# fxxJuses/MICFormer

Measured on AMD Instinct MI355X. Metric: train volumes/sec (128^3 CT+MRI pair), higher is better.
Workload: dtype bf16; 1 GPU; MicFormer base Head(embed_dim=48, depths 2-2-6-2, heads 3-6-12-24, window 2^3, 8 classes) full train step (fwd + MDiceLoss + bwd + Adam/cosine) on 128^3 CT+MR pairs, DropPath on; local_batch=2, global_batch=2, parallelism=dp1, launch=hipGraph replay (one graph)

## Files before the change

### micformer_amd/csrc/common.h

```cpp
#pragma once
#include <hip/hip_runtime.h>
#include <stdint.h>

#include "../../include/micformer_hip.h"
#include "gemm_core.h"

#define MICF_RETURN_LAUNCH()                          \
  do {                                                \
    return hipGetLastError() == hipSuccess ? MICF_OK : MICF_ELAUNCH; \
  } while (0)

namespace micf {

struct Options {
  int block_wave = 1;
  int block_recompute_h = 0;
  int block_debug = 0;
  int sample_tile = 1;
  int sample_e = -1;
  int cell_cap = -1;
  int tile_cap_hits = -1, tile_cap_cell = -1, tile_cap_voxel = -1;
};
Options& options();

struct Geo {
  int B, D, H, W;
  FastDiv fW, fH, fD;
  Geo() {}
  Geo(int B_, int D_, int H_, int W_) : B(B_), D(D_), H(H_), W(W_), fW((uint32_t)W_), fH((uint32_t)H_), fD((uint32_t)D_) {}
  __host__ __device__ int64_t tokens() const { return (int64_t)B * D * H * W; }
  __device__ __forceinline__ void decode(int t, int& b, int& d, int& h, int& w) const {
    uint32_t q, r;
    fW.divmod((uint32_t)t, q, r); w = (int)r;
    fH.divmod(q, q, r); h = (int)r;
    fD.divmod(q, q, r); d = (int)r; b = (int)q;
  }
  __device__ __forceinline__ int token(int b, int d, int h, int w) const { return ((b * D + d) * H + h) * W + w; }
};

__device__ __forceinline__ float wave_sum(float v) {
#pragma unroll
  for (int o = 32; o > 0; o >>= 1) v += __shfl_xor(v, o, 64);
  return v;
}

int colsum_atomic(const float* dy, const float* scale, int64_t rps, float* out, int64_t M, int N, hipStream_t s);

constexpr int kOffsetHidden = 16;
struct CellLists {
  int* count;
  int* ovf_count;
  int* list;
  int* ovf;
  int cap;
  float* w8;
};
struct SampleFwdSet { const float *h, *ln_g, *ln_b, *w1, *xa; float *flow, *xs; };
struct SampleBwdSet {
  const float *dxs, *h, *ln_g, *ln_b, *w1, *xa, *flow;
  float *dxa, *dh, *dln_g, *dln_b, *dw1;
  CellLists cl;
  float* partials;
};
int offset_sample_fwd_groups(const SampleFwdSet* sets, int n, int B, int D, int H, int W, int C, float eps, hipStream_t stream);
int offset_sample_bwd_groups(SampleBwdSet* sets, int n, int B, int D, int H, int W, int C, float eps, float* workspace,
                             int64_t workspace_floats, hipStream_t s, int phase = 0);
struct SampleFinishCall { const SampleBwdSet* sets; int n, B, D, H, W, C; float* workspace; int64_t workspace_floats; };
int offset_sample_finish_many(const SampleFinishCall* calls, int ncalls, hipStream_t s);

struct Conv3FwdSet { const float* x1; const float* x2; const float* w; const float* bias; float* y; float* wt; };
struct Conv3BwdSet { const float* dy; const float* w; float* wt; float* dx1; float* dx2; };
int conv3_fwd_x_groups(const Conv3FwdSet* sets, int n, int c1, int c2, int B, int D, int H, int W, int N, hipStream_t stream, int dtype,
                       int prepared, int y_zeroed);
bool conv3_fwd_x_splits(int B, int D, int H, int W, int c1, int c2);
int conv3_bwd_data_x_groups(const Conv3BwdSet* sets, int ng, int c1, int acc1, int c2, int acc2, int B, int D, int H, int W, int N,
                            hipStream_t stream, int dtype, int prepared);

int conv3_bwd_data_x(const float* dy, const float* w, float* wt, float* dx1, int c1, int acc1, float* dx2, int c2, int acc2, int B,
                     int D, int H, int W, int N, hipStream_t stream, int dtype = 0, int prepared = 0);

int64_t conv3_fwdx_workspace(int N, int c1, int c2);
int conv3_fwd_x(const float* x1, int c1, const float* x2, int c2, const float* w, const float* bias, float* y, float* wt, int B, int D,
                int H, int W, int N, hipStream_t stream, int dtype = 0, int prepared = 0);
int64_t conv3_wgradx_workspace(int B, int D, int H, int W, int N, int c1, int c2, int items = 1);
int conv3_wgradx_items(const float* const* dy, const float* const* x1, const float* const* x2, float* const* dw, float* const* dbias,
                       int n, int c1, int c2, int B, int D, int H, int W, int N, float* ws, int64_t ws_floats, hipStream_t stream,
                       int dtype);
int conv3_wgradx(const float* dy, const float* x1, int c1, const float* x2, int c2, float* dw, float* dbias, int B, int D, int H,
                 int W, int N, float* ws, int64_t ws_floats, hipStream_t stream, int dtype = 0);

}
```

### micformer_amd/csrc/conv3_bwdx.hip

```cpp
#include <cstdlib>
#include "common.h"
#include "conv3_layout.h"
#include "gemm_dma.h"

namespace micf {

constexpr int xKS = 20;

struct BwdxArgs {
  const float* dy; int N;
  const float* wt;
  float* d1; float* d2; int oc1, oc2, acc1, acc2;
  int O;
  int B, D, H, W, tiles_d, tiles_h, tiles_w, ngroups;
  const float* dyb; const float* wtb; float* d1b; float* d2b;
};

__global__ void __launch_bounds__(256) conv3_wt_kernel(const float* __restrict__ w, float* __restrict__ wt, int N, int Cin) {
  const int64_t id = (int64_t)blockIdx.x * 256 + threadIdx.x;
  if (id < conv3_bwd_layout_items(Cin)) conv3_bwd_layout_write(w, wt, N, Cin, id);
}

template <int TW, int NCT, bool BF16>
__global__ void __launch_bounds__(256) conv3_bwdx_kernel(BwdxArgs a) {
  constexpr int CH = 16 / TW, TH = 4 * CH, TD = 2;
  constexpr int HD = TD + 2, HH = TH + 2, HW = TW + 2, HALO = HD * HH * HW;
  __shared__ __attribute__((aligned(16))) float Xs[HALO * xKS];
  if (blockIdx.z) { a.dy = a.dyb; a.wt = a.wtb; a.d1 = a.d1b; a.d2 = a.d2b; }
  const int tid = threadIdx.x, lane = tid & 63, wave = __builtin_amdgcn_readfirstlane(tid >> 6), li = lane & 15, lr = lane >> 4;
  int q = blockIdx.x;
  if (gridDim.x >= 64 && (gridDim.x & 7) == 0) q = (q & 7) * (gridDim.x >> 3) + (q >> 3);
  const int tw = q % a.tiles_w; q /= a.tiles_w;
  const int th = q % a.tiles_h; q /= a.tiles_h;
  const int td = q % a.tiles_d; const int b = q / a.tiles_d;
  const int d0 = td * TD, h0 = th * TH, w0 = tw * TW;
  const int64_t DHW = (int64_t)a.D * a.H * a.W;
  const int ct0 = blockIdx.y * NCT;
  const int nct = min(NCT, a.O / 16 - ct0);

  {
    constexpr int NH = (HALO * 4 + 255) / 256;
    float4 hv4[NH];
#pragma unroll
    for (int it = 0; it < NH; ++it) {
      const int idx = tid + it * 256;
      hv4[it] = make_float4(0.f, 0.f, 0.f, 0.f);
      if (idx < HALO * 4) {
        const int hv = idx >> 2, g = idx & 3;
        const int hw = hv % HW, hh = (hv / HW) % HH, hd = hv / (HW * HH);
        const int dd = d0 + hd - 1, yy = h0 + hh - 1, ww = w0 + hw - 1;
        if ((unsigned)dd < (unsigned)a.D && (unsigned)yy < (unsigned)a.H && (unsigned)ww < (unsigned)a.W && 4 * g < a.N)
          hv4[it] = *reinterpret_cast<const float4*>(a.dy + ((int64_t)b * DHW + ((int64_t)dd * a.H + yy) * a.W + ww) * a.N + 4 * g);
      }
    }
#pragma unroll
    for (int it = 0; it < NH; ++it) {
      const int idx = tid + it * 256;
      if (idx < HALO * 4) {
        if constexpr (BF16)
          *reinterpret_cast<uint2*>(&reinterpret_cast<uint16_t*>(Xs)[(idx >> 2) * xKS + 4 * (idx & 3)]) =
              make_uint2(pack_bf16(hv4[it].x, hv4[it].y), pack_bf16(hv4[it].z, hv4[it].w));
        else
          *reinterpret_cast<float4*>(&Xs[(idx >> 2) * xKS + 4 * (idx & 3)]) = hv4[it];
      }
    }
  }
  int ld[2], lh[2], lw[2];
#pragma unroll
  for (int tj = 0; tj < 2; ++tj) {
    const int ct = 2 * wave + tj;
    ld[tj] = ct / 4;
    lh[tj] = (ct % 4) * CH + li / TW;
    lw[tj] = li % TW;
  }
  f32x4 acc[NCT][2];
#pragma unroll
  for (int t = 0; t < NCT; ++t) { acc[t][0] = f32x4{0.f, 0.f, 0.f, 0.f}; acc[t][1] = f32x4{0.f, 0.f, 0.f, 0.f}; }
  const float* wp = a.wt + ((int64_t)(ct0 * 16 + li)) * 16 + 4 * lr;
  const int64_t tap_stride = (int64_t)a.O * 16;
  if constexpr (BF16) {
    typedef unsigned u32x4 __attribute__((ext_vector_type(4)));
    const uint16_t* Xh = reinterpret_cast<const uint16_t*>(Xs);
    const u32x4* wq = reinterpret_cast<const u32x4*>(reinterpret_cast<const uint16_t*>(a.wt + conv3_bwd_layout_f32(a.O)) +
                                                     (((int64_t)(ct0 * 16 + li)) * 4 + lr) * 8);
    const int64_t pair_stride = (int64_t)a.O * 4;
// ... 64 lines not shown
  for (int t = 0; t < NCT; ++t) av[t] = (t < nct && !BF16) ? *reinterpret_cast<const float4*>(wp + t * 256) : make_float4(0.f, 0.f, 0.f, 0.f);
  if constexpr (!BF16) __syncthreads();
#pragma unroll 1
  for (int tap = 0; tap < (BF16 ? 0 : 27); ++tap) {
    if (tap + 1 < 27) {
#pragma unroll
      for (int t = 0; t < NCT; ++t)
        an[t] = (t < nct) ? *reinterpret_cast<const float4*>(wp + (tap + 1) * tap_stride + t * 256) : make_float4(0.f, 0.f, 0.f, 0.f);
    }
    const int kd = tap / 9, kh = (tap / 3) % 3, kw = tap % 3;
    float4 bv[2];
#pragma unroll
    for (int tj = 0; tj < 2; ++tj) {
      const int zd = ld[tj] + 2 - kd, zh = lh[tj] + 2 - kh, zw = lw[tj] + 2 - kw;
      bv[tj] = *reinterpret_cast<const float4*>(&Xs[((zd * HH + zh) * HW + zw) * xKS + 4 * lr]);
    }
    if constexpr (!BF16) {
#pragma unroll
      for (int s = 0; s < 4; ++s) {
        const float b0 = s == 0 ? bv[0].x : (s == 1 ? bv[0].y : (s == 2 ? bv[0].z : bv[0].w));
        const float b1 = s == 0 ? bv[1].x : (s == 1 ? bv[1].y : (s == 2 ? bv[1].z : bv[1].w));
#pragma unroll
        for (int t = 0; t < NCT; ++t) {
          const float av_s = s == 0 ? av[t].x : (s == 1 ? av[t].y : (s == 2 ? av[t].z : av[t].w));
          acc[t][0] = __builtin_amdgcn_mfma_f32_16x16x4f32(av_s, b0, acc[t][0], 0, 0, 0);
          acc[t][1] = __builtin_amdgcn_mfma_f32_16x16x4f32(av_s, b1, acc[t][1], 0, 0, 0);
        }
      }
    } else {
      if ((tap & 1) || tap == 26) {
        const float4 z = make_float4(0.f, 0.f, 0.f, 0.f);
        const bool pair = tap & 1;
        const bf16x8 bb0 = pair ? to_bf16x8(bprev[0], bv[0]) : to_bf16x8(bv[0], z);
        const bf16x8 bb1 = pair ? to_bf16x8(bprev[1], bv[1]) : to_bf16x8(bv[1], z);
#pragma unroll
        for (int t = 0; t < NCT; ++t) {
          const bf16x8 ba = pair ? to_bf16x8(aprev[t], av[t]) : to_bf16x8(av[t], z);
          acc[t][0] = __builtin_amdgcn_mfma_f32_16x16x32_bf16(ba, bb0, acc[t][0], 0, 0, 0);
          acc[t][1] = __builtin_amdgcn_mfma_f32_16x16x32_bf16(ba, bb1, acc[t][1], 0, 0, 0);
        }
      } else {
        bprev[0] = bv[0]; bprev[1] = bv[1];
#pragma unroll
        for (int t = 0; t < NCT; ++t) aprev[t] = av[t];
      }
    }
#pragma unroll
    for (int t = 0; t < NCT; ++t) av[t] = an[t];
  }
#pragma unroll
  for (int tj = 0; tj < 2; ++tj) {
    const int dd = d0 + ld[tj], yy = h0 + lh[tj], ww = w0 + lw[tj];
    if (dd >= a.D || yy >= a.H || ww >= a.W) continue;
    const int64_t tok = (int64_t)b * DHW + ((int64_t)dd * a.H + yy) * a.W + ww;
    auto where = [&](int t, int& accf) -> float* {
      const int c = (ct0 + t) * 16 + 4 * lr;
      if (t >= nct) return nullptr;
      if (c < a.oc1) { accf = a.acc1; return a.d1 ? a.d1 + tok * a.oc1 + c : nullptr; }
      accf = a.acc2;
      return a.d2 ? a.d2 + tok * a.oc2 + (c - a.oc1) : nullptr;
    };
    constexpr int EB = NCT >= 6 ? 2 : NCT;
#pragma unroll
    for (int t0 = 0; t0 < NCT; t0 += EB) {
      float4 old[EB];
#pragma unroll
      for (int u = 0; u < EB; ++u) {
        int accf = 0;
        const float* p = where(t0 + u, accf);
        old[u] = (p && accf) ? *reinterpret_cast<const float4*>(p) : make_float4(0.f, 0.f, 0.f, 0.f);
      }
#pragma unroll
      for (int u = 0; u < EB; ++u) {
        int accf = 0;
        float* p = where(t0 + u, accf);
        if (!p) continue;
        const f32x4 v = acc[t0 + u][tj];
        *reinterpret_cast<float4*>(p) = make_float4(v[0] + old[u].x, v[1] + old[u].y, v[2] + old[u].z, v[3] + old[u].w);
      }
    }
  }
}

template <int TW, bool BF16>
static hipError_t launch_bwdx(BwdxArgs& a, hipStream_t stream) {
  constexpr int CH = 16 / TW, TH = 4 * CH;
  a.tiles_d = (a.D + 1) / 2;
  a.tiles_h = (a.H + TH - 1) / TH;
  a.tiles_w = (a.W + TW - 1) / TW;
  const int64_t blocks = (int64_t)a.B * a.tiles_d * a.tiles_h * a.tiles_w;
  const int cts = a.O / 16;
  if (blocks * ((cts + 5) / 6) >= 128)
    hipLaunchKernelGGL((conv3_bwdx_kernel<TW, 6, BF16>), dim3((unsigned)blocks, (cts + 5) / 6, a.ngroups), dim3(256), 0, stream, a);
  else
    hipLaunchKernelGGL((conv3_bwdx_kernel<TW, 2, BF16>), dim3((unsigned)blocks, (cts + 1) / 2, a.ngroups), dim3(256), 0, stream, a);
  return hipGetLastError();
}

int conv3_bwd_data_x(const float* dy, const float* w, float* wt, float* dx1, int c1, int acc1, float* dx2, int c2, int acc2, int B,
                     int D, int H, int W, int N, hipStream_t stream, int dtype, int prepared) {
  const Conv3BwdSet one{dy, w, wt, dx1, dx2};
  return conv3_bwd_data_x_groups(&one, 1, c1, acc1, c2, acc2, B, D, H, W, N, stream, dtype, prepared);
}

int conv3_bwd_data_x_groups(const Conv3BwdSet* sets, int ng, int c1, int acc1, int c2, int acc2, int B, int D, int H, int W, int N,
                            hipStream_t stream, int dtype, int prepared) {
  if (!sets || ng < 1 || ng > 2) return MICF_EINVAL;
  const int O = c1 + c2;
  if (N > 16 || (N & 3) || (O & 15) || (c1 & 3) || (c2 & 3) || W < 4) return MICF_EUNSUPPORTED;
  for (int i = 0; i < ng; ++i)
    if (!aligned16(sets[i].dy) || !aligned16(sets[i].wt) || (sets[i].dx1 && !aligned16(sets[i].dx1)) || (sets[i].dx2 && !aligned16(sets[i].dx2)) ||
        (!sets[i].dx1) != (!sets[0].dx1) || (!sets[i].dx2) != (!sets[0].dx2))
      return MICF_EUNSUPPORTED;
  const float *dy = sets[0].dy;
  float *wt = sets[0].wt, *dx1 = sets[0].dx1, *dx2 = sets[0].dx2;
  const int64_t n = conv3_bwd_layout_items(O);
  if (!prepared) {
    for (int i = 0; i < ng; ++i) {
      hipLaunchKernelGGL(conv3_wt_kernel, dim3((unsigned)((n + 255) / 256)), dim3(256), 0, stream, sets[i].w, sets[i].wt, N, O);
      if (hipGetLastError() != hipSuccess) return MICF_ELAUNCH;
    }
  }
  BwdxArgs a{};
  a.dyb = sets[ng - 1].dy; a.wtb = sets[ng - 1].wt; a.d1b = sets[ng - 1].dx1; a.d2b = sets[ng - 1].dx2; a.ngroups = ng;
  a.dy = dy; a.N = N; a.wt = wt; a.d1 = dx1; a.d2 = dx2; a.oc1 = c1; a.oc2 = c2; a.acc1 = acc1; a.acc2 = acc2; a.O = O;
  a.B = B; a.D = D; a.H = H; a.W = W;
  const hipError_t e = dtype == MICF_DTYPE_BF16 ? ((W >= 12) ? launch_bwdx<16, true>(a, stream) : launch_bwdx<8, true>(a, stream))
                                                 : ((W >= 12) ? launch_bwdx<16, false>(a, stream) : launch_bwdx<8, false>(a, stream));
  return e == hipSuccess ? MICF_OK : MICF_ELAUNCH;
}

}
```

### micformer_amd/csrc/conv3_fwdx.hip

```cpp
#include <cstdlib>
#include "common.h"
#include "conv3_layout.h"
#include "gemm_dma.h"

namespace micf {

constexpr int fKS = 20;
constexpr int fAhead = 3;

struct FwdxArgs {
  const float* x1; const float* x2; int c1, c2;
  const float* wt;
  const float* bias; float* y; int N;
  const float* x1b; const float* x2b; const float* wtb; const float* biasb; float* yb;
  int B, D, H, W, tiles_d, tiles_h, tiles_w;
  int chunks, chunks_per_block;
};

__global__ void __launch_bounds__(256) conv3_wtf_kernel(const float* __restrict__ w, float* __restrict__ wt, int N, int Cin, int chunks) {
  const int64_t id = (int64_t)blockIdx.x * 256 + threadIdx.x;
  if (id < conv3_fwd_layout_items(Cin)) conv3_fwd_layout_write(w, wt, N, Cin, id);
}

template <int TW, bool BF16>
__global__ void __launch_bounds__(256) conv3_fwdx_kernel(FwdxArgs a) {
  constexpr int CH = 16 / TW, TH = 4 * CH, TD = 2;
  constexpr int HD = TD + 2, HH = TH + 2, HW = TW + 2, HALO = HD * HH * HW;
  constexpr int NH = (HALO * 4 + 255) / 256;
  __shared__ __attribute__((aligned(16))) float Xs[HALO * fKS];
  if (blockIdx.z) { a.x1 = a.x1b; a.x2 = a.x2b; a.wt = a.wtb; a.bias = a.biasb; a.y = a.yb; }
  const int tid = threadIdx.x, lane = tid & 63, wave = __builtin_amdgcn_readfirstlane(tid >> 6), li = lane & 15, lr = lane >> 4;
  int q = blockIdx.x;
  if (gridDim.x >= 64 && (gridDim.x & 7) == 0) q = (q & 7) * (gridDim.x >> 3) + (q >> 3);
  const int tw = q % a.tiles_w; q /= a.tiles_w;
  const int th = q % a.tiles_h; q /= a.tiles_h;
  const int td = q % a.tiles_d; const int b = q / a.tiles_d;
  const int d0 = td * TD, h0 = th * TH, w0 = tw * TW;
  const int64_t DHW = (int64_t)a.D * a.H * a.W;
  const int Cin = a.c1 + a.c2;
  const int kc_begin = blockIdx.y * a.chunks_per_block;
  const int kc_end = min(a.chunks, kc_begin + a.chunks_per_block);

  auto fetch = [&](int kc, float4 (&hv)[NH]) {
#pragma unroll
    for (int it = 0; it < NH; ++it) {
      const int idx = tid + it * 256;
      hv[it] = make_float4(0.f, 0.f, 0.f, 0.f);
      if (idx < HALO * 4) {
        const int v = idx >> 2, g = idx & 3;
        const int hw = v % HW, hh = (v / HW) % HH, hd = v / (HW * HH);
        const int dd = d0 + hd - 1, yy = h0 + hh - 1, ww = w0 + hw - 1;
        const int c = kc * 16 + 4 * g;
        if ((unsigned)dd < (unsigned)a.D && (unsigned)yy < (unsigned)a.H && (unsigned)ww < (unsigned)a.W && c < Cin) {
          const int64_t tok = (int64_t)b * DHW + ((int64_t)dd * a.H + yy) * a.W + ww;
          hv[it] = c < a.c1 ? *reinterpret_cast<const float4*>(a.x1 + tok * a.c1 + c)
                            : *reinterpret_cast<const float4*>(a.x2 + tok * a.c2 + (c - a.c1));
        }
      }
    }
  };
  uint16_t* Xh = reinterpret_cast<uint16_t*>(Xs);
  auto commit = [&](const float4 (&hv)[NH]) {
#pragma unroll
    for (int it = 0; it < NH; ++it) {
      const int idx = tid + it * 256;
      if (idx < HALO * 4) {
        if constexpr (BF16)
          *reinterpret_cast<uint2*>(&Xh[(idx >> 2) * fKS + 4 * (idx & 3)]) = make_uint2(pack_bf16(hv[it].x, hv[it].y), pack_bf16(hv[it].z, hv[it].w));
        else
          *reinterpret_cast<float4*>(&Xs[(idx >> 2) * fKS + 4 * (idx & 3)]) = hv[it];
      }
    }
  };

  int vbase[2];
#pragma unroll
  for (int tj = 0; tj < 2; ++tj) {
    const int ct = 2 * wave + tj;
    const int ld = ct / 4, lh = (ct % 4) * CH + li / TW, lw = li % TW;
    vbase[tj] = ((ld * HH + lh) * HW + lw) * fKS + 4 * lr;
  }
  f32x4 acc[2] = {f32x4{0.f, 0.f, 0.f, 0.f}, f32x4{0.f, 0.f, 0.f, 0.f}};
  float4 hv[NH];
  fetch(kc_begin, hv);
  for (int kc = kc_begin; kc < kc_end; ++kc) {
// ... 17 lines not shown
#pragma unroll
        for (int e = 0; e < 2; ++e) {
          const int tap = 2 * p + e;
          if (tap < 27) {
            const int kd = tap / 9, kh = (tap / 3) % 3, kw = tap % 3;
            const int off = ((kd * HH + kh) * HW + kw) * fKS;
            h[e][0] = *reinterpret_cast<const uint2*>(&Xh[vbase[0] + off]);
            h[e][1] = *reinterpret_cast<const uint2*>(&Xh[vbase[1] + off]);
          } else {
            h[e][0] = make_uint2(0u, 0u); h[e][1] = h[e][0];
          }
        }
        const u32x4 q0 = {h[0][0].x, h[0][0].y, h[1][0].x, h[1][0].y}, q1 = {h[0][1].x, h[0][1].y, h[1][1].x, h[1][1].y};
        acc[0] = __builtin_amdgcn_mfma_f32_16x16x32_bf16(__builtin_bit_cast(bf16x8, aq), __builtin_bit_cast(bf16x8, q0), acc[0], 0, 0, 0);
        acc[1] = __builtin_amdgcn_mfma_f32_16x16x32_bf16(__builtin_bit_cast(bf16x8, aq), __builtin_bit_cast(bf16x8, q1), acc[1], 0, 0, 0);
      }
      continue;
    }
    float4 ring[fAhead + 1];
    float4 aprev = make_float4(0.f, 0.f, 0.f, 0.f);
    uint2 hprev0 = make_uint2(0u, 0u), hprev1 = hprev0;
#pragma unroll
    for (int t = 0; t < fAhead; ++t) ring[t] = *reinterpret_cast<const float4*>(wp + t * 256);
#pragma unroll
    for (int tap = 0; tap < 27; ++tap) {
      if (tap + fAhead < 27) ring[(tap + fAhead) % (fAhead + 1)] = *reinterpret_cast<const float4*>(wp + (tap + fAhead) * 256);
      const float4 av = ring[tap % (fAhead + 1)];
      const int kd = tap / 9, kh = (tap / 3) % 3, kw = tap % 3;
      const int off = ((kd * HH + kh) * HW + kw) * fKS;
      if constexpr (!BF16) {
        const float4 b0 = *reinterpret_cast<const float4*>(&Xs[vbase[0] + off]);
        const float4 b1 = *reinterpret_cast<const float4*>(&Xs[vbase[1] + off]);
        acc[0] = __builtin_amdgcn_mfma_f32_16x16x4f32(av.x, b0.x, acc[0], 0, 0, 0);
        acc[1] = __builtin_amdgcn_mfma_f32_16x16x4f32(av.x, b1.x, acc[1], 0, 0, 0);
        acc[0] = __builtin_amdgcn_mfma_f32_16x16x4f32(av.y, b0.y, acc[0], 0, 0, 0);
        acc[1] = __builtin_amdgcn_mfma_f32_16x16x4f32(av.y, b1.y, acc[1], 0, 0, 0);
        acc[0] = __builtin_amdgcn_mfma_f32_16x16x4f32(av.z, b0.z, acc[0], 0, 0, 0);
        acc[1] = __builtin_amdgcn_mfma_f32_16x16x4f32(av.z, b1.z, acc[1], 0, 0, 0);
        acc[0] = __builtin_amdgcn_mfma_f32_16x16x4f32(av.w, b0.w, acc[0], 0, 0, 0);
        acc[1] = __builtin_amdgcn_mfma_f32_16x16x4f32(av.w, b1.w, acc[1], 0, 0, 0);
      } else {
        typedef unsigned u32x4 __attribute__((ext_vector_type(4)));
        const uint2 h0 = *reinterpret_cast<const uint2*>(&Xh[vbase[0] + off]);
        const uint2 h1 = *reinterpret_cast<const uint2*>(&Xh[vbase[1] + off]);
        if ((tap & 1) || tap == 26) {
          const float4 z = make_float4(0.f, 0.f, 0.f, 0.f);
          const bool pair = tap & 1;
          const bf16x8 ba = pair ? to_bf16x8(aprev, av) : to_bf16x8(av, z);
          const u32x4 q0 = pair ? u32x4{hprev0.x, hprev0.y, h0.x, h0.y} : u32x4{h0.x, h0.y, 0u, 0u};
          const u32x4 q1 = pair ? u32x4{hprev1.x, hprev1.y, h1.x, h1.y} : u32x4{h1.x, h1.y, 0u, 0u};
          acc[0] = __builtin_amdgcn_mfma_f32_16x16x32_bf16(ba, __builtin_bit_cast(bf16x8, q0), acc[0], 0, 0, 0);
          acc[1] = __builtin_amdgcn_mfma_f32_16x16x32_bf16(ba, __builtin_bit_cast(bf16x8, q1), acc[1], 0, 0, 0);
        } else {
          aprev = av; hprev0 = h0; hprev1 = h1;
        }
      }
    }
  }
  const bool atomic_out = gridDim.y > 1;
  const int n0 = 4 * lr;
#pragma unroll
  for (int tj = 0; tj < 2; ++tj) {
    const int ct = 2 * wave + tj;
    const int dd = d0 + ct / 4, yy = h0 + (ct % 4) * CH + li / TW, ww = w0 + li % TW;
    if (dd >= a.D || yy >= a.H || ww >= a.W || n0 >= a.N) continue;
    float* p = a.y + ((int64_t)b * DHW + ((int64_t)dd * a.H + yy) * a.W + ww) * a.N + n0;
    f32x4 v = acc[tj];
    if (a.bias && blockIdx.y == 0) {
#pragma unroll
      for (int e = 0; e < 4; ++e) if (n0 + e < a.N) v[e] += a.bias[n0 + e];
    }
    if (atomic_out) {
#pragma unroll
      for (int e = 0; e < 4; ++e) if (n0 + e < a.N) atomicAdd(p + e, v[e]);
    } else if (n0 + 3 < a.N && (a.N & 3) == 0) {
      *reinterpret_cast<float4*>(p) = make_float4(v[0], v[1], v[2], v[3]);
    } else {
#pragma unroll
      for (int e = 0; e < 4; ++e) if (n0 + e < a.N) p[e] = v[e];
    }
  }
}

int64_t conv3_fwdx_workspace(int N, int c1, int c2) {
  if (N <= 0 || N > 16 || c1 + c2 <= 0) return 0;
  return conv3_fwd_layout_floats(c1 + c2);
}

int conv3_fwd_x(const float* x1, int c1, const float* x2, int c2, const float* w, const float* bias, float* y, float* wt, int B, int D,
                int H, int W, int N, hipStream_t stream, int dtype, int prepared) {
  const Conv3FwdSet one{x1, x2, w, bias, y, wt};
  return conv3_fwd_x_groups(&one, 1, c1, c2, B, D, H, W, N, stream, dtype, prepared, 0);
}

bool conv3_fwd_x_splits(int B, int D, int H, int W, int c1, int c2) {
  const int chunks = (c1 + c2 + 15) / 16;
  const int tw_ = W >= 12 ? 16 : 8, th_ = 4 * (16 / tw_);
  const int64_t blocks = (int64_t)B * ((D + 1) / 2) * ((H + th_ - 1) / th_) * ((W + tw_ - 1) / tw_);
  return blocks < 256 && chunks > 1;
}

int conv3_fwd_x_groups(const Conv3FwdSet* sets, int n, int c1, int c2, int B, int D, int H, int W, int N, hipStream_t stream, int dtype,
                       int prepared, int y_zeroed) {
  if (!sets || n < 1 || n > 2) return MICF_EINVAL;
  if (N > 16 || (c1 & 3) || (c2 & 3) || W < 4) return MICF_EUNSUPPORTED;
  for (int i = 0; i < n; ++i)
    if (!aligned16(sets[i].x1) || (sets[i].x2 && !aligned16(sets[i].x2)) || !aligned16(sets[i].y) || !aligned16(sets[i].wt)) return MICF_EUNSUPPORTED;
  const float *x1 = sets[0].x1, *x2 = sets[0].x2, *w = sets[0].w, *bias = sets[0].bias;
  float *y = sets[0].y, *wt = sets[0].wt;
  const int Cin = c1 + c2, chunks = (Cin + 15) / 16;
  const int64_t nw = conv3_fwd_layout_items(Cin);
  if (!prepared) {
    for (int i = 0; i < n; ++i) {
      hipLaunchKernelGGL(conv3_wtf_kernel, dim3((unsigned)((nw + 255) / 256)), dim3(256), 0, stream, sets[i].w, sets[i].wt, N, Cin, chunks);
      if (hipGetLastError() != hipSuccess) return MICF_ELAUNCH;
    }
  }
  FwdxArgs a{};
  a.x1 = x1; a.x2 = x2 ? x2 : x1; a.c1 = c1; a.c2 = c2; a.wt = wt; a.bias = bias; a.y = y; a.N = N;
  a.B = B; a.D = D; a.H = H; a.W = W; a.chunks = chunks;
  const Conv3FwdSet& sb = sets[n - 1];
  a.x1b = sb.x1; a.x2b = sb.x2 ? sb.x2 : sb.x1; a.wtb = sb.wt; a.biasb = sb.bias; a.yb = sb.y;
  const int tw_ = W >= 12 ? 16 : 8, th_ = 4 * (16 / tw_);
  a.tiles_d = (D + 1) / 2; a.tiles_h = (H + th_ - 1) / th_; a.tiles_w = (W + tw_ - 1) / tw_;
  const int64_t blocks = (int64_t)B * a.tiles_d * a.tiles_h * a.tiles_w;
  int ysplit = 1;
  constexpr int split_target = 128;
  if (blocks < 256) { ysplit = (int)((split_target + blocks - 1) / blocks); if (ysplit > chunks) ysplit = chunks; if (ysplit < 1) ysplit = 1; }
  a.chunks_per_block = (chunks + ysplit - 1) / ysplit;
  ysplit = (chunks + a.chunks_per_block - 1) / a.chunks_per_block;
  if (ysplit > 1 && !y_zeroed)
    for (int i = 0; i < n; ++i)
      if (hipMemsetAsync(sets[i].y, 0, sizeof(float) * (size_t)B * D * H * W * N, stream) != hipSuccess) return MICF_ELAUNCH;
  const dim3 grid((unsigned)blocks, ysplit, n);
  if (dtype == MICF_DTYPE_BF16) {
    if (tw_ == 16) hipLaunchKernelGGL((conv3_fwdx_kernel<16, true>), grid, dim3(256), 0, stream, a);
    else hipLaunchKernelGGL((conv3_fwdx_kernel<8, true>), grid, dim3(256), 0, stream, a);
  } else {
    if (tw_ == 16) hipLaunchKernelGGL((conv3_fwdx_kernel<16, false>), grid, dim3(256), 0, stream, a);
    else hipLaunchKernelGGL((conv3_fwdx_kernel<8, false>), grid, dim3(256), 0, stream, a);
  }
  return hipGetLastError() == hipSuccess ? MICF_OK : MICF_ELAUNCH;
}

}
```

### micformer_amd/csrc/misc.hip

```cpp
#include <hip/hip_fp16.h>

#include "common.h"
#include <string.h>

namespace micf {

__global__ void __launch_bounds__(256) pad3d_kernel(const float* __restrict__ src, float* __restrict__ dst, int B, int D, int H,
                                                    int W, int Dp, int Hp, int Wp, int C, int64_t total) {
  for (int64_t i = (int64_t)blockIdx.x * 256 + threadIdx.x; i < total; i += (int64_t)gridDim.x * 256) {
    int64_t t = i / C; const int c = (int)(i - t * C);
    const int w = (int)(t % Wp); t /= Wp; const int h = (int)(t % Hp); t /= Hp; const int d = (int)(t % Dp); const int b = (int)(t / Dp);
    dst[i] = (d < D && h < H && w < W) ? src[((((int64_t)b * D + d) * H + h) * W + w) * C + c] : 0.f;
  }
}
__global__ void __launch_bounds__(256) crop3d_kernel(const float* __restrict__ src, float* __restrict__ dst, int B, int D, int H,
                                                     int W, int Dp, int Hp, int Wp, int C, int accumulate, int64_t total) {
  for (int64_t i = (int64_t)blockIdx.x * 256 + threadIdx.x; i < total; i += (int64_t)gridDim.x * 256) {
    int64_t t = i / C; const int c = (int)(i - t * C);
    const int w = (int)(t % W); t /= W; const int h = (int)(t % H); t /= H; const int d = (int)(t % D); const int b = (int)(t / D);
    const float v = src[((((int64_t)b * Dp + d) * Hp + h) * Wp + w) * C + c];
    dst[i] = accumulate ? dst[i] + v : v;
  }
}

__device__ __forceinline__ void ac_coord(int o, int Sin, int Sout, int& i0, int& i1, float& f) {
  const float scale = Sout > 1 ? (float)(Sin - 1) / (float)(Sout - 1) : 0.f;
  const float s = scale * (float)o;
  i0 = (int)s; if (i0 > Sin - 1) i0 = Sin - 1;
  i1 = i0 + (i0 < Sin - 1 ? 1 : 0);
  f = s - (float)i0;
}
template <bool BWD>
__global__ void __launch_bounds__(256) resize_kernel(const float* __restrict__ a, float* __restrict__ o, int B, int D, int H, int W,
                                                     int Do, int Ho, int Wo, int C, int64_t total) {
  for (int64_t i = (int64_t)blockIdx.x * 256 + threadIdx.x; i < total; i += (int64_t)gridDim.x * 256) {
    int64_t t = i / C; const int c = (int)(i - t * C);
    const int w = (int)(t % Wo); t /= Wo; const int h = (int)(t % Ho); t /= Ho; const int d = (int)(t % Do); const int b = (int)(t / Do);
    int d0, d1, h0, h1, w0, w1; float fd, fh, fw;
    ac_coord(d, D, Do, d0, d1, fd); ac_coord(h, H, Ho, h0, h1, fh); ac_coord(w, W, Wo, w0, w1, fw);
    float acc = 0.f;
    const float gv = BWD ? a[i] : 0.f;
#pragma unroll
    for (int q = 0; q < 8; ++q) {
      const int dd = (q & 4) ? d1 : d0, hh = (q & 2) ? h1 : h0, ww = (q & 1) ? w1 : w0;
      const float wt = ((q & 4) ? fd : 1.f - fd) * ((q & 2) ? fh : 1.f - fh) * ((q & 1) ? fw : 1.f - fw);
      const int64_t s = ((((int64_t)b * D + dd) * H + hh) * W + ww) * C + c;
      if (BWD) atomicAdd(o + s, wt * gv); else acc += wt * a[s];
    }
    if (!BWD) o[i] = acc;
  }
}

}
using namespace micf;

extern "C" int micf_abi_version(void) { return MICF_ABI_VERSION; }

micf::Options& micf::options() {
  static Options o;
  return o;
}

static int* option_slot(const char* name) {
  if (!name) return nullptr;
  Options& o = micf::options();
  const struct { const char* n; int* v; } table[] = {
      {"block_wave", &o.block_wave}, {"block_recompute_h", &o.block_recompute_h}, {"block_debug", &o.block_debug},
      {"sample_tile", &o.sample_tile}, {"sample_e", &o.sample_e}, {"cell_cap", &o.cell_cap},
      {"tile_cap_hits", &o.tile_cap_hits}, {"tile_cap_cell", &o.tile_cap_cell}, {"tile_cap_voxel", &o.tile_cap_voxel}};
  for (const auto& e : table)
    if (!strcmp(name, e.n)) return e.v;
  return nullptr;
}

extern "C" int micf_set_option(const char* name, int value) {
  int* slot = option_slot(name);
  if (!slot) return MICF_EINVAL;
  *slot = value;
  return MICF_OK;
}

extern "C" int micf_get_option(const char* name, int* value) {
  const int* slot = option_slot(name);
  if (!slot || !value) return MICF_EINVAL;
  *value = *slot;
  return MICF_OK;
}

extern "C" const char* micf_strerror(int code) {
  switch (code) {
    case MICF_OK: return "ok";
    case MICF_EINVAL: return "invalid argument (null pointer, bad size or misaligned buffer)";
    case MICF_EUNSUPPORTED: return "shape not supported by the HIP kernels";
    case MICF_ELAUNCH: return "HIP kernel launch failed";
    default: return "unknown micf error code";
  }
}

static int grid_for(int64_t total) { int64_t b = (total + 255) / 256; return (int)(b > 16384 ? 16384 : (b < 1 ? 1 : b)); }

extern "C" int micf_pad3d(const float* src, float* dst, int B, int D, int H, int W, int Dp, int Hp, int Wp, int C,
                          micf_stream_t stream) {
  if (!src || !dst || B <= 0 || D <= 0 || H <= 0 || W <= 0 || C <= 0 || Dp < D || Hp < H || Wp < W) return MICF_EINVAL;
  const int64_t total = (int64_t)B * Dp * Hp * Wp * C;
  hipLaunchKernelGGL(pad3d_kernel, dim3(grid_for(total)), dim3(256), 0, (hipStream_t)stream, src, dst, B, D, H, W, Dp, Hp, Wp, C, total);
  MICF_RETURN_LAUNCH();
}
extern "C" int micf_crop3d(const float* src, float* dst, int B, int D, int H, int W, int Dp, int Hp, int Wp, int C, int accumulate,
                           micf_stream_t stream) {
  if (!src || !dst || B <= 0 || D <= 0 || H <= 0 || W <= 0 || C <= 0 || Dp < D || Hp < H || Wp < W) return MICF_EINVAL;
  const int64_t total = (int64_t)B * D * H * W * C;
  hipLaunchKernelGGL(crop3d_kernel, dim3(grid_for(total)), dim3(256), 0, (hipStream_t)stream, src, dst, B, D, H, W, Dp, Hp, Wp, C,
                     accumulate, total);
  MICF_RETURN_LAUNCH();
}
extern "C" int micf_resize_trilinear_fwd(const float* src, float* dst, int B, int D, int H, int W, int Do, int Ho, int Wo, int C,
                                         micf_stream_t stream) {
  if (!src || !dst || B <= 0 || D <= 0 || H <= 0 || W <= 0 || Do <= 0 || Ho <= 0 || Wo <= 0 || C <= 0) return MICF_EINVAL;
  const int64_t total = (int64_t)B * Do * Ho * Wo * C;
  hipLaunchKernelGGL(resize_kernel<false>, dim3(grid_for(total)), dim3(256), 0, (hipStream_t)stream, src, dst, B, D, H, W, Do, Ho, Wo, C, total);
  MICF_RETURN_LAUNCH();
}
extern "C" int micf_resize_trilinear_bwd(const float* ddst, float* dsrc, int B, int D, int H, int W, int Do, int Ho, int Wo, int C,
                                         micf_stream_t stream) {
  if (!ddst || !dsrc || B <= 0 || D <= 0 || H <= 0 || W <= 0 || Do <= 0 || Ho <= 0 || Wo <= 0 || C <= 0) return MICF_EINVAL;
  hipStream_t s = (hipStream_t)stream;
  if (hipMemsetAsync(dsrc, 0, sizeof(float) * (size_t)B * D * H * W * C, s) != hipSuccess) return MICF_ELAUNCH;
  const int64_t total = (int64_t)B * Do * Ho * Wo * C;
  hipLaunchKernelGGL(resize_kernel<true>, dim3(grid_for(total)), dim3(256), 0, s, ddst, dsrc, B, D, H, W, Do, Ho, Wo, C, total);
  MICF_RETURN_LAUNCH();
}

extern "C" int micf_zero(void* p, int64_t bytes, micf_stream_t stream) {
  if (!p || bytes < 0) return MICF_EINVAL;
  if (bytes == 0) return MICF_OK;
  return hipMemsetAsync(p, 0, (size_t)bytes, (hipStream_t)stream) == hipSuccess ? MICF_OK : MICF_ELAUNCH;
}

namespace micf {
__device__ __forceinline__ uint64_t mix64(uint64_t z) {
  z += 0x9E3779B97F4A7C15ull;
  z = (z ^ (z >> 30)) * 0xBF58476D1CE4E5B9ull;
  z = (z ^ (z >> 27)) * 0x94D049BB133111EBull;
  return z ^ (z >> 31);
}
__global__ void __launch_bounds__(256) drop_path_draw_kernel(uint64_t* __restrict__ rng, const float* __restrict__ keep,
                                                             float* __restrict__ out, int n, int B) {
  const uint64_t seed = rng[0], ctr = rng[1];
  for (int e = threadIdx.x; e < n * B; e += 256) {
    const float k = keep[e / B];
    const uint64_t h = mix64(mix64(seed ^ mix64(ctr)) + (uint64_t)e);
    const float u = (float)(h >> 40) * (1.0f / 16777216.0f);
// ... 239 lines not shown
```

Before: 243.2 pairs/s.

## Add depth-marching 3x3x3 conv forward and backward-data kernels with LDS plane ring

Adds new conv3 forward and backward-data kernels. Each workgroup owns a 4x16 spatial footprint and marches along depth, keeping a three-plane bf16 halo ring in LDS, so each input plane is fetched once and reused across the three kd taps. Weights are held in registers for the whole march and the 27 taps are fed as MFMA 16x16x32 bf16 with double-buffered LDS reads. A plan header splits depth into ranges so the grid fills the chip and orders units for XCD locality. The new path is chosen automatically when bf16, N==16 and the grid is large enough, with a fallback to the old kernels and an option to disable it; the risks are lower occupancy from the larger LDS and extra synchronisation per depth step.

After: 243.5 pairs/s (median of 3 runs). No clear change (+0.1%).

```diff
diff --git a/micformer_amd/csrc/common.h b/micformer_amd/csrc/common.h
--- a/micformer_amd/csrc/common.h
+++ b/micformer_amd/csrc/common.h
@@ -20,6 +20,9 @@
   int sample_e = -1;
   int cell_cap = -1;
   int tile_cap_hits = -1, tile_cap_cell = -1, tile_cap_voxel = -1;
+  int conv3_march = -1;
+  int conv3_march_dcap = -1;
+  int conv3_march_last = 0;
 };
 Options& options();
 
diff --git a/micformer_amd/csrc/conv3_bwdx.hip b/micformer_amd/csrc/conv3_bwdx.hip
--- a/micformer_amd/csrc/conv3_bwdx.hip
+++ b/micformer_amd/csrc/conv3_bwdx.hip
@@ -1,6 +1,7 @@
 #include <cstdlib>
 #include "common.h"
 #include "conv3_layout.h"
+#include "conv3_march_plan.h"
 #include "gemm_dma.h"
 
 namespace micf {
@@ -231,6 +232,166 @@
   }
 }
 
+namespace mp = micf_march;
+constexpr int mDYB = 40;
+constexpr int mThreads = 64 * mp::kWaves;
+
+struct BwdMarchArgs {
+  const float* dy; const float* wt; float* d1; float* d2;
+  const float* dyb; const float* wtb; float* d1b; float* d2b;
+  int oc1, oc2, acc1, acc2, O;
+  mp::Plan plan;
+};
+
+__global__ void __launch_bounds__(mThreads, 3) conv3_bwdx_march_kernel(BwdMarchArgs a) {
+  typedef unsigned u32x4 __attribute__((ext_vector_type(4)));
+  constexpr int HW = mp::kHaloW, PL = mp::kPlaneRows, PLB = PL * mDYB;
+  constexpr int NQ = PL * 4;
+  constexpr int NB = (NQ + mThreads - 1) / mThreads;
+  __shared__ __attribute__((aligned(16))) char ring[3 * PLB];
+  if (blockIdx.z) { a.dy = a.dyb; a.wt = a.wtb; a.d1 = a.d1b; a.d2 = a.d2b; }
+  const int tid = threadIdx.x, lane = tid & 63, wave = __builtin_amdgcn_readfirstlane(tid >> 6), li = lane & 15, lr = lane >> 4;
+  const mp::Unit un = mp::decode(a.plan, blockIdx.x);
+  const int D = a.plan.D, H = a.plan.H, W = a.plan.W, h0 = un.h0, w0 = un.w0;
+  const int64_t tok0 = (int64_t)un.b * D * H * W;
+  const int tile = blockIdx.y * mp::kWaves + wave;
+  const bool active = tile * 16 < a.O;
+
+  const float* fsrc[NB];
+  unsigned fdst[NB];
+  unsigned fok = 0u;
+#pragma unroll
+  for (int u = 0; u < NB; ++u) {
+    const int idx = u * mThreads + tid, hv = idx >> 2, g = idx & 3;
+    const int yy = h0 + hv / HW - 1, ww = w0 + hv % HW - 1;
+    const bool ok = idx < NQ && (unsigned)yy < (unsigned)H && (unsigned)ww < (unsigned)W;
+    fsrc[u] = a.dy + (tok0 + (ok ? (int64_t)yy * W + ww : 0)) * 16 + 4 * g;
+    fdst[u] = (unsigned)(hv * mDYB + 8 * g);
+    fok |= ok ? 1u << u : 0u;
+  }
+  const int64_t fstride = (int64_t)H * W * 16;
+  auto fetch = [&](int dd, float4 (&v)[NB]) {
+    if ((unsigned)dd < (unsigned)D) {
+#pragma unroll
+      for (int u = 0; u < NB; ++u) v[u] = *reinterpret_cast<const float4*>(fsrc[u] + dd * fstride);
+    } else {
+#pragma unroll
+      for (int u = 0; u < NB; ++u) v[u] = make_float4(0.f, 0.f, 0.f, 0.f);
+    }
+  };
+  auto commit = [&](int slot, const float4 (&v)[NB]) {
+#pragma unroll
+    for (int u = 0; u < NB; ++u)
+      if (u * mThreads + tid < NQ) {
+        const bool ok = (fok >> u) & 1u;
+        *reinterpret_cast<uint2*>(ring + slot * PLB + fdst[u]) =
+            ok ? make_uint2(pack_bf16(v[u].x, v[u].y), pack_bf16(v[u].z, v[u].w)) : make_uint2(0u, 0u);
+      }
+  };
+
+  float4 va[NB], vb[NB];
+  int sc = un.d0 % 3;
+  {
+    float4 p0[NB], p1[NB];
+    fetch(un.d0 - 1, p0);
+    fetch(un.d0, p1);
+    fetch(un.d0 + 1, va);
+    if (un.d0 + 1 < un.d1) fetch(un.d0 + 2, vb);
+    commit(sc == 0 ? 2 : sc - 1, p0);
+    commit(sc, p1);
+  }
+  u32x4 aq[14];
+  {
+    const u32x4 zq = {0u, 0u, 0u, 0u};
+    const u32x4* wq = reinterpret_cast<const u32x4*>(reinterpret_cast<const uint16_t*>(a.wt + conv3_bwd_layout_f32(a.O))) +
+                      (((int64_t)(active ? tile : 0) * 16 + li) * 4 + lr);
+    const int64_t pair_stride = (int64_t)a.O * 4;
+#pragma unroll
+    for (int p = 0; p < 14; ++p) aq[p] = active ? wq[p * pair_stride] : zq;
+  }
+  float* outp = nullptr;
+  int ocw = 0, oacc = 0;
+  if (active && w0 + li < W) {
+    const int c = tile * 16 + 4 * lr;
+    const int64_t t = tok0 + (int64_t)h0 * W + w0 + li;
+    if (c < a.oc1) { ocw = a.oc1; oacc = a.acc1; outp = a.d1 ? a.d1 + t * a.oc1 + c : nullptr; }
+    else { ocw = a.oc2; oacc = a.acc2; outp = a.d2 ? a.d2 + t * a.oc2 + (c - a.oc1) : nullptr; }
+  }
+  const int64_t orow = (int64_t)W * ocw;
+  const unsigned lbase = (unsigned)(li * mDYB + 8 * lr);
+
+  auto step = [&](int d, float4 (&v)[NB]) {
+    const int sp = sc == 0 ? 2 : sc - 1, sn = sc == 2 ? 0 : sc + 1;
+    __syncthreads();
+    commit(sn, v);
+    __syncthreads();
+    if (d + 2 < un.d1) fetch(d + 3, v);
+    if (active) {
+      float* const op = outp ? outp + (int64_t)d * H * orow : nullptr;
+      float4 old[mp::kFootH];
+#pragma unroll
+      for (int j = 0; j < mp::kFootH; ++j) {
+        old[j] = make_float4(0.f, 0.f, 0.f, 0.f);
+        if (op && oacc && h0 + j < H) old[j] = *reinterpret_cast<const float4*>(op + j * orow);
+      }
+      const char* pk[3] = {ring + sn * PLB + lbase, ring + sc * PLB + lbase, ring + sp * PLB + lbase};
+      f32x4 acc[mp::kFootH];
+#pragma unroll
+      for (int j = 0; j < mp::kFootH; ++j) acc[j] = f32x4{0.f, 0.f, 0.f, 0.f};
+      auto read_stage = [&](int st, u32x4 (&bq)[2]) {
+        const int p = st >> 1;
+#pragma unroll
+        for (int jj = 0; jj < 2; ++jj) {
+          const int j = 2 * (st & 1) + jj;
+          uint2 h[2];
+#pragma unroll
+          for (int e = 0; e < 2; ++e) {
+            const int tap = 2 * p + e;
+            h[e] = make_uint2(0u, 0u);
+            if (tap < 27) {
+              const int kd = tap / 9, kh = (tap / 3) % 3, kw = tap % 3;
+              h[e] = *reinterpret_cast<const uint2*>(pk[kd] + ((j + 2 - kh) * HW + 2 - kw) * mDYB);
+            }
+          }
+          bq[jj] = u32x4{h[0].x, h[0].y, h[1].x, h[1].y};
+        }
+      };
+      u32x4 bq[2][2];
+      read_stage(0, bq[0]);
+#pragma unroll
+      for (int st = 0; st < 28; ++st) {
+        if (st + 1 < 28) read_stage(st + 1, bq[(st + 1) & 1]);
+#pragma unroll
+        for (int jj = 0; jj < 2; ++jj) {
+          const int j = 2 * (st & 1) + jj;
+          acc[j] = __builtin_amdgcn_mfma_f32_16x16x32_bf16(__builtin_bit_cast(bf16x8, aq[st >> 1]), __builtin_bit_cast(bf16x8, bq[st & 1][jj]), acc[j], 0, 0, 0);
+        }
+        __builtin_amdgcn_sched_barrier(0);
+      }
+      if (op) {
+#pragma unroll
+        for (int j = 0; j < mp::kFootH; ++j)
+          if (h0 + j < H)
+            *reinterpret_cast<float4*>(op + j * orow) =
+                make_float4(acc[j][0] + old[j].x, acc[j][1] + old[j].y, acc[j][2] + old[j].z, acc[j][3] + old[j].w);
+      }
+    }
+    sc = sn;
+  };
+  for (int d = un.d0; d < un.d1; d += 2) {
+    step(d, va);
+    if (d + 1 < un.d1) step(d + 1, vb);
+  }
+}
+
+static bool bwdx_marches(int ng, int O, int B, int D, int H, int W, int N, int dtype, mp::Plan& plan, int& ysplit) {
+  const Options& opt = options();
+  if (dtype != MICF_DTYPE_BF16 || opt.conv3_march == 0 || N != 16 || (int64_t)H * W * O > 0x7fffffffll) return false;
+  ysplit = (O / 16 + mp::kWaves - 1) / mp::kWaves;
+  plan = mp::make_plan(B, D, H, W, ng * ysplit, opt.conv3_march_dcap);
+  return opt.conv3_march == 1 || (W >= 12 && mp::fills_chip(plan, ng * ysplit));
+}
+
 template <int TW, bool BF16>
 static hipError_t launch_bwdx(BwdxArgs& a, hipStream_t stream) {
   constexpr int CH = 16 / TW, TH = 4 * CH;
@@ -270,6 +431,20 @@
       if (hipGetLastError() != hipSuccess) return MICF_ELAUNCH;
     }
   }
+  options().conv3_march_last = 0;
+  {
+    BwdMarchArgs m{};
+    int ysplit = 1;
+    if (bwdx_marches(ng, O, B, D, H, W, N, dtype, m.plan, ysplit)) {
+      m.dy = dy; m.wt = wt; m.d1 = dx1; m.d2 = dx2;
+      m.dyb = sets[ng - 1].dy; m.wtb = sets[ng - 1].wt; m.d1b = sets[ng - 1].dx1; m.d2b = sets[ng - 1].dx2;
+      m.oc1 = c1; m.oc2 = c2; m.acc1 = acc1; m.acc2 = acc2; m.O = O;
+      hipLaunchKernelGGL(conv3_bwdx_march_kernel, dim3((unsigned)m.plan.units, ysplit, ng), dim3(mThreads), 0, stream, m);
+      if (hipGetLastError() != hipSuccess) return MICF_ELAUNCH;
+      options().conv3_march_last = 1;
+      return MICF_OK;
+    }
+  }
   BwdxArgs a{};
   a.dyb = sets[ng - 1].dy; a.wtb = sets[ng - 1].wt; a.d1b = sets[ng - 1].dx1; a.d2b = sets[ng - 1].dx2; a.ngroups = ng;
   a.dy = dy; a.N = N; a.wt = wt; a.d1 = dx1; a.d2 = dx2; a.oc1 = c1; a.oc2 = c2; a.acc1 = acc1; a.acc2 = acc2; a.O = O;
diff --git a/micformer_amd/csrc/conv3_fwdx.hip b/micformer_amd/csrc/conv3_fwdx.hip
--- a/micformer_amd/csrc/conv3_fwdx.hip
+++ b/micformer_amd/csrc/conv3_fwdx.hip
@@ -1,6 +1,8 @@
 #include <cstdlib>
+#include <mutex>
 #include "common.h"
 #include "conv3_layout.h"
+#include "conv3_march_plan.h"
 #include "gemm_dma.h"
 
 namespace micf {
@@ -184,6 +186,180 @@
   }
 }
 
+namespace mp = micf_march;
+template <int NW> constexpr int mf_red_bytes() { return (NW / 2) * mp::kFootH * 64 * 16; }
+template <int NW> constexpr int mf_row_bytes() { return 2 * 16 * NW + 16; }
+template <int NW> constexpr int mf_lds_bytes() { return 3 * mp::kPlaneRows * mf_row_bytes<NW>() + mf_red_bytes<NW>(); }
+
+struct FwdMarchArgs {
+  const float* x1; const float* x2; const float* wt; const float* bias; float* y;
+  const float* x1b; const float* x2b; const float* wtb; const float* biasb; float* yb;
+  int c1, c2;
+  mp::Plan plan;
+};
+
+template <int NW>
+__global__ void __launch_bounds__(64 * NW, 3) conv3_fwdx_march_kernel(FwdMarchArgs a) {
+  typedef unsigned u32x4 __attribute__((ext_vector_type(4)));
+  constexpr int HW = mp::kHaloW, PL = mp::kPlaneRows, RS = mf_row_bytes<NW>(), PLB = PL * RS, mfThreads = 64 * NW;
+  constexpr int NB = (PL * 4 * NW + mfThreads - 1) / mfThreads;
+  extern __shared__ __attribute__((aligned(16))) char mf_smem[];
+  char* const ring = mf_smem;
+  float4* const red = reinterpret_cast<float4*>(mf_smem + 3 * PLB);
+  if (blockIdx.z) { a.x1 = a.x1b; a.x2 = a.x2b; a.wt = a.wtb; a.bias = a.biasb; a.y = a.yb; }
+  const int tid = threadIdx.x, lane = tid & 63, wave = __builtin_amdgcn_readfirstlane(tid >> 6), li = lane & 15, lr = lane >> 4;
+  const mp::Unit un = mp::decode(a.plan, blockIdx.x);
+  const int D = a.plan.D, H = a.plan.H, W = a.plan.W, h0 = un.h0, w0 = un.w0;
+  const int64_t tok0 = (int64_t)un.b * D * H * W;
+  const int Cin = a.c1 + a.c2, chunks = Cin >> 4;
+
+  const int G = Cin >> 2, RP = mfThreads / G, g = tid % G, r0 = tid / G;
+  const bool first = 4 * g < a.c1;
+  const int cw = first ? a.c1 : a.c2;
+  const float* const fbase = (first ? a.x1 + 4 * g : a.x2 + (4 * g - a.c1)) + tok0 * cw;
+  const int64_t fstride = (int64_t)H * W * cw;
+  const unsigned fdst = (unsigned)(r0 * RS + 8 * g);
+  unsigned foff[NB];
+  unsigned fok = 0u;
+#pragma unroll
+  for (int u = 0; u < NB; ++u) {
+    const int hv = u * RP + r0;
+    const int yy = h0 + hv / HW - 1, ww = w0 + hv % HW - 1;
+    const bool ok = hv < PL && (unsigned)yy < (unsigned)H && (unsigned)ww < (unsigned)W;
+    foff[u] = ok ? (unsigned)((yy * W + ww) * cw) : 0u;
+    fok |= ok ? 1u << u : 0u;
+  }
+  auto fetch = [&](int dd, float4 (&v)[NB]) {
+    if ((unsigned)dd < (unsigned)D) {
+      const float* const src = fbase + dd * fstride;
+#pragma unroll
+      for (int u = 0; u < NB; ++u) v[u] = *reinterpret_cast<const float4*>(src + (size_t)foff[u]);
+    } else {
+#pragma unroll
+      for (int u = 0; u < NB; ++u) v[u] = make_float4(0.f, 0.f, 0.f, 0.f);
+    }
+  };
+  auto commit = [&](int slot, const float4 (&v)[NB]) {
+#pragma unroll
+    for (int u = 0; u < NB; ++u)
+      if (u * RP + r0 < PL) {
+        const bool ok = (fok >> u) & 1u;
+        *reinterpret_cast<uint2*>(ring + slot * PLB + fdst + u * RP * RS) =
+            ok ? make_uint2(pack_bf16(v[u].x, v[u].y), pack_bf16(v[u].z, v[u].w)) : make_uint2(0u, 0u);
+      }
+  };
+
+  float4 v[NB];
+  int sc = un.d0 % 3;
+  {
+    float4 p0[NB];
+    fetch(un.d0 - 1, p0);
+    fetch(un.d0, v);
+    commit(sc == 0 ? 2 : sc - 1, p0);
+    commit(sc, v);
+    fetch(un.d0 + 1, v);
+  }
+  const bool active = wave < chunks;
+  u32x4 aq[14];
+  {
+    const u32x4 zq = {0u, 0u, 0u, 0u};
+    const u32x4* wq = reinterpret_cast<const u32x4*>(reinterpret_cast<const uint16_t*>(a.wt + conv3_fwd_layout_f32(Cin))) +
+                      (((int64_t)(active ? wave : 0) * 14 * 16 + li) * 4 + lr);
+#pragma unroll
+    for (int p = 0; p < 14; ++p) aq[p] = active ? wq[p * 64] : zq;
+  }
+  float* yp = nullptr;
+  float4 bias4 = make_float4(0.f, 0.f, 0.f, 0.f);
+  if (wave < mp::kFootH && h0 + wave < H && w0 + li < W) {
+    yp = a.y + (tok0 + (int64_t)(h0 + wave) * W + w0 + li) * 16 + 4 * lr;
+    if (a.bias) bias4 = make_float4(a.bias[4 * lr], a.bias[4 * lr + 1], a.bias[4 * lr + 2], a.bias[4 * lr + 3]);
+  }
+  const int64_t ystride = (int64_t)H * W * 16;
+  auto finish = [&](int d) {
+    if (wave < mp::kFootH) {
+      float4 s = red[wave * 64 + lane];
+#pragma unroll
+      for (int i = 1; i < NW / 2; ++i) {
+        const float4 t = red[(i * mp::kFootH + wave) * 64 + lane];
+        s.x += t.x; s.y += t.y; s.z += t.z; s.w += t.w;
+      }
+      if (yp) *reinterpret_cast<float4*>(yp + d * ystride) = make_float4(s.x + bias4.x, s.y + bias4.y, s.z + bias4.z, s.w + bias4.w);
+    }
+  };
+  const unsigned lbase = (unsigned)(li * RS + 8 * lr + wave * 32);
+
+  for (int d = un.d0; d < un.d1; ++d) {
+    const int sp = sc == 0 ? 2 : sc - 1, sn = sc == 2 ? 0 : sc + 1;
+    __syncthreads();
+    commit(sn, v);
+    if (d > un.d0) finish(d - 1);
+    __syncthreads();
+    if (d + 1 < un.d1) fetch(d + 2, v);
+    f32x4 acc[mp::kFootH];
+#pragma unroll
+    for (int j = 0; j < mp::kFootH; ++j) acc[j] = f32x4{0.f, 0.f, 0.f, 0.f};
+    if (active) {
+      const char* pk[3] = {ring + sp * PLB + lbase, ring + sc * PLB + lbase, ring + sn * PLB + lbase};
+      auto read_stage = [&](int st, u32x4 (&bq)[2]) {
+        const int p = st >> 1;
+#pragma unroll
+        for (int jj = 0; jj < 2; ++jj) {
+          const int j = 2 * (st & 1) + jj;
+          uint2 h[2];
+#pragma unroll
+          for (int e = 0; e < 2; ++e) {
+            const int tap = 2 * p + e;
+            h[e] = make_uint2(0u, 0u);
+            if (tap < 27) {
+              const int kd = tap / 9, kh = (tap / 3) % 3, kw = tap % 3;
+              h[e] = *reinterpret_cast<const uint2*>(pk[kd] + ((j + kh) * HW + kw) * RS);
+            }
+          }
+          bq[jj] = u32x4{h[0].x, h[0].y, h[1].x, h[1].y};
+        }
+      };
+      u32x4 bq[2][2];
+      read_stage(0, bq[0]);
+#pragma unroll
+      for (int st = 0; st < 28; ++st) {
+        if (st + 1 < 28) read_stage(st + 1, bq[(st + 1) & 1]);
+#pragma unroll
+        for (int jj = 0; jj < 2; ++jj) {
+          const int j = 2 * (st & 1) + jj;
+          acc[j] = __builtin_amdgcn_mfma_f32_16x16x32_bf16(__builtin_bit_cast(bf16x8, aq[st >> 1]), __builtin_bit_cast(bf16x8, bq[st & 1][jj]), acc[j], 0, 0, 0);
+        }
+        __builtin_amdgcn_sched_barrier(0);
+      }
+    }
+    if (wave >= NW / 2) {
+#pragma unroll
+      for (int j = 0; j < mp::kFootH; ++j) red[((wave - NW / 2) * mp::kFootH + j) * 64 + lane] = make_float4(acc[j][0], acc[j][1], acc[j][2], acc[j][3]);
+    }
+    __syncthreads();
+    if (wave < NW / 2) {
+#pragma unroll
+      for (int j = 0; j < mp::kFootH; ++j) {
+        float4& r = red[(wave * mp::kFootH + j) * 64 + lane];
+        const float4 o = r;
+        r = make_float4(acc[j][0] + o.x, acc[j][1] + o.y, acc[j][2] + o.z, acc[j][3] + o.w);
+      }
+    }
+    sc = sn;
+  }
+  __syncthreads();
+  finish(un.d1 - 1);
+}
+
+static bool fwdx_marches(int n, int c1, int c2, int B, int D, int H, int W, int N, int dtype, mp::Plan& plan) {
+  const Options& opt = options();
+  const int Cin = c1 + c2, cmax = c1 > c2 ? c1 : c2;
+  if (dtype != MICF_DTYPE_BF16 || opt.conv3_march == 0 || N != 16 || Cin <= 0 || (Cin & 15) || Cin > 192 || (64 * (Cin <= 96 ? 6 : 12)) % (Cin / 4) ||
+      (int64_t)H * W * (cmax > 16 ? cmax : 16) > 0x7fffffffll)
+    return false;
+  plan = mp::make_plan(B, D, H, W, n, opt.conv3_march_dcap);
+  return opt.conv3_march == 1 || (W >= 12 && mp::fills_chip(plan, n));
+}
+
 int64_t conv3_fwdx_workspace(int N, int c1, int c2) {
   if (N <= 0 || N > 16 || c1 + c2 <= 0) return 0;
   return conv3_fwd_layout_floats(c1 + c2);
@@ -216,6 +392,27 @@
     for (int i = 0; i < n; ++i) {
       hipLaunchKernelGGL(conv3_wtf_kernel, dim3((unsigned)((nw + 255) / 256)), dim3(256), 0, stream, sets[i].w, sets[i].wt, N, Cin, chunks);
       if (hipGetLastError() != hipSuccess) return MICF_ELAUNCH;
+    }
+  }
+  options().conv3_march_last = 0;
+  {
+    FwdMarchArgs m{};
+    if (fwdx_marches(n, c1, c2, B, D, H, W, N, dtype, m.plan)) {
+      const Conv3FwdSet& s1 = sets[n - 1];
+      m.x1 = x1; m.x2 = x2 ? x2 : x1; m.wt = wt; m.bias = bias; m.y = y;
+      m.x1b = s1.x1; m.x2b = s1.x2 ? s1.x2 : s1.x1; m.wtb = s1.wt; m.biasb = s1.bias; m.yb = s1.y;
+      m.c1 = c1; m.c2 = c2;
+      static std::once_flag attr_once;
+      std::call_once(attr_once, [] {
+        (void)hipFuncSetAttribute(reinterpret_cast<const void*>(&conv3_fwdx_march_kernel<6>), hipFuncAttributeMaxDynamicSharedMemorySize, mf_lds_bytes<6>());
+        (void)hipFuncSetAttribute(reinterpret_cast<const void*>(&conv3_fwdx_march_kernel<12>), hipFuncAttributeMaxDynamicSharedMemorySize, mf_lds_bytes<12>());
+      });
+      const dim3 mgrid((unsigned)m.plan.units, 1, n);
+      if (chunks <= 6) hipLaunchKernelGGL((conv3_fwdx_march_kernel<6>), mgrid, dim3(64 * 6), (mf_lds_bytes<6>()), stream, m);
+      else hipLaunchKernelGGL((conv3_fwdx_march_kernel<12>), mgrid, dim3(64 * 12), (mf_lds_bytes<12>()), stream, m);
+      if (hipGetLastError() != hipSuccess) return MICF_ELAUNCH;
+      options().conv3_march_last = 1;
+      return MICF_OK;
     }
   }
   FwdxArgs a{};
diff --git a/micformer_amd/csrc/conv3_march_plan.h b/micformer_amd/csrc/conv3_march_plan.h
--- /dev/null
+++ b/micformer_amd/csrc/conv3_march_plan.h
@@ -0,0 +1,70 @@
+#pragma once
+#include <stdint.h>
+
+#if defined(__HIPCC__) || defined(__CUDACC__)
+#define MICF_MARCH_HD __host__ __device__ inline
+#else
+#define MICF_MARCH_HD inline
+#endif
+
+namespace micf_march {
+
+constexpr int kFootH = 4, kFootW = 16;
+constexpr int kHaloH = kFootH + 2, kHaloW = kFootW + 2;
+constexpr int kPlaneRows = kHaloH * kHaloW;
+constexpr int kWaves = 6;
+constexpr int kWgTarget = 512;
+constexpr int kWgFill = 128;
+constexpr int kMinRange = 2;
+
+struct Plan {
+  int B, D, H, W;
+  int tiles_h, tiles_w;
+  int nranges;
+  int units;
+  int xcd_order;
+};
+
+struct Unit { int b, h0, w0, d0, d1; };
+
+MICF_MARCH_HD Plan make_plan(int B, int D, int H, int W, int mult, int cap) {
+  Plan p;
+  p.B = B; p.D = D; p.H = H; p.W = W;
+  p.tiles_h = (H + kFootH - 1) / kFootH;
+  p.tiles_w = (W + kFootW - 1) / kFootW;
+  const int64_t base = (int64_t)B * p.tiles_h * p.tiles_w * (mult > 0 ? mult : 1);
+  const int64_t want = (kWgTarget + base - 1) / base;
+  const int most = D / kMinRange > 1 ? D / kMinRange : 1;
+  int n = (int)(want < most ? want : most);
+  if (cap > 0 && (D + cap - 1) / cap > n) n = (D + cap - 1) / cap;
+  p.nranges = n;
+  p.units = B * p.tiles_h * p.tiles_w * n;
+  p.xcd_order = p.units % 8 == 0 ? 1 : 0;
+  return p;
+}
+
+MICF_MARCH_HD int range_begin(const Plan& p, int r) { return (int)((int64_t)r * p.D / p.nranges); }
+
+MICF_MARCH_HD bool fills_chip(const Plan& p, int mult) { return (int64_t)p.units * mult >= kWgFill; }
+
+MICF_MARCH_HD Unit decode(const Plan& p, int lin) {
+  int q = p.xcd_order ? (lin % 8) * (p.units / 8) + lin / 8 : lin;
+  Unit u;
+  const int r = q % p.nranges; q /= p.nranges;
+  u.w0 = (q % p.tiles_w) * kFootW; q /= p.tiles_w;
+  u.h0 = (q % p.tiles_h) * kFootH;
+  u.b = q / p.tiles_h;
+  u.d0 = range_begin(p, r);
+  u.d1 = range_begin(p, r + 1);
+  return u;
+}
+
+MICF_MARCH_HD bool zero_plane(const Plan& p, int d) { return d < 0 || d >= p.D; }
+
+MICF_MARCH_HD int64_t slot_token(const Plan& p, const Unit& u, int d, int slot) {
+  const int h = u.h0 + slot / kFootW, w = u.w0 + slot % kFootW;
+  if (h >= p.H || w >= p.W) return -1;
+  return (((int64_t)u.b * p.D + d) * p.H + h) * p.W + w;
+}
+
+}
diff --git a/micformer_amd/csrc/misc.hip b/micformer_amd/csrc/misc.hip
--- a/micformer_amd/csrc/misc.hip
+++ b/micformer_amd/csrc/misc.hip
@@ -67,7 +67,8 @@
   const struct { const char* n; int* v; } table[] = {
       {"block_wave", &o.block_wave}, {"block_recompute_h", &o.block_recompute_h}, {"block_debug", &o.block_debug},
       {"sample_tile", &o.sample_tile}, {"sample_e", &o.sample_e}, {"cell_cap", &o.cell_cap},
-      {"tile_cap_hits", &o.tile_cap_hits}, {"tile_cap_cell", &o.tile_cap_cell}, {"tile_cap_voxel", &o.tile_cap_voxel}};
+      {"tile_cap_hits", &o.tile_cap_hits}, {"tile_cap_cell", &o.tile_cap_cell}, {"tile_cap_voxel", &o.tile_cap_voxel},
+      {"conv3_march", &o.conv3_march}, {"conv3_march_dcap", &o.conv3_march_dcap}, {"conv3_march_last", &o.conv3_march_last}};
   for (const auto& e : table)
     if (!strcmp(name, e.n)) return e.v;
   return nullptr;
```
